# bupt-ai-cz/HIAST

Measured on AMD Instinct MI355X. Metric: self-training images/sec (fwd+bwd+pseudo-label) at 1024x512, higher is better.
Workload: dtype fp16

## Files before the change

hiast_amd/csrc/igemm.hip:

```cpp
#include "igemm_kernel.h"

namespace hiast {

template <int PL>
__device__ __forceinline__ size_t ig_wp_elem(int n, int t, int k, int taps, int KO)
{
    const size_t row = ((size_t)n * taps + t) * PL * KO;
    return PL == 2 ? row + (size_t)(k >> 5) * 64 + (k & 31) : row + k;
}

template <int PL, bool F16 = false>
__global__ __launch_bounds__(256) void pack_conv_weight_kernel(const float* __restrict__ w,
                                                               unsigned short* __restrict__ wp,
                                                               unsigned short* __restrict__ wpt, int N, int K, int taps,
                                                               int mode)
{
    const long long idx = (long long)blockIdx.x * 256 + threadIdx.x;
    if (idx >= (long long)N * taps * K) return;
    const int k = (int)(idx % K);
    const int t = (int)((idx / K) % taps);
    const int n = (int)(idx / ((long long)K * taps));
    const float v = w[((size_t)n * K + k) * taps + t];
    unsigned short h, l = 0;
    if (F16) h = H16<true>::enc(v);
    else ig_split(v, h, l);
    if (mode != 1) {
        unsigned short* d = wp + ig_wp_elem<PL>(n, t, k, taps, K);
        d[0] = h;
        if (PL == 2) d[32] = l;
    }
    if (mode != 0) {
        unsigned short* d = (mode == 1 ? wp : wpt) + ig_wp_elem<PL>(k, taps - 1 - t, n, taps, N);
        d[0] = h;
        if (PL == 2) d[32] = l;
    }
}

constexpr int PK_PITCH = 72;

template <int PL, bool F16 = false>
__device__ __forceinline__ void pack_tile(const float* __restrict__ w, unsigned short* __restrict__ wp,
                                          unsigned short* __restrict__ wpt, int N, int K, int taps, int mode, int n0,
                                          int k0, unsigned short* lds)
{
    constexpr int TN = PL == 1 ? 32 : 16;
    unsigned short* hi = lds;
    unsigned short* lo = lds + (PL == 2 ? TN * taps * PK_PITCH : 0);
    unsigned short* fwd = (mode == 1) ? nullptr : wp;
    unsigned short* adj = (mode == 0) ? nullptr : (mode == 1 ? wp : wpt);
    const int run = 64 * taps;
    for (int nh = 0; nh < 64; nh += TN) {
        if (nh) __syncthreads();
        for (int e = threadIdx.x; e < TN * run; e += 256) {
            const int n = e / run, r = e - n * run;
            const int k = r / taps, t = r - k * taps;
            const float v = w[((size_t)(n0 + nh + n) * K + k0) * taps + r];
            unsigned short h, l = 0;
            if (F16) h = H16<true>::enc(v);
            else ig_split(v, h, l);
            hi[(n * taps + t) * PK_PITCH + k] = h;
            if (PL == 2) lo[(n * taps + t) * PK_PITCH + k] = l;
        }
        __syncthreads();
        if (fwd) {
            for (int e = threadIdx.x; e < TN * taps * 8; e += 256) {
                const int c = e & 7, nt = e >> 3;
                const int n = nt / taps, t = nt - n * taps;
                const uint4 vh = *reinterpret_cast<const uint4*>(&hi[nt * PK_PITCH + c * 8]);
                unsigned short* d = fwd + ig_wp_elem<PL>(n0 + nh + n, t, k0 + c * 8, taps, K);
                *reinterpret_cast<uint4*>(d) = vh;
                if (PL == 2) *reinterpret_cast<uint4*>(d + 32) = *reinterpret_cast<const uint4*>(&lo[nt * PK_PITCH + c * 8]);
            }
        }
        if (adj) {
            for (int e = threadIdx.x; e < 64 * taps * (TN / 8); e += 256) {
                const int c = e % (TN / 8), kt = e / (TN / 8);
                const int k = kt / taps, t = kt - k * taps;
                unsigned short vh[8], vl[8];
#pragma unroll
                for (int j = 0; j < 8; ++j) {
                    vh[j] = hi[((c * 8 + j) * taps + t) * PK_PITCH + k];
                    if (PL == 2) vl[j] = lo[((c * 8 + j) * taps + t) * PK_PITCH + k];
                }
                unsigned short* d = adj + ig_wp_elem<PL>(k0 + k, taps - 1 - t, n0 + nh + c * 8, taps, N);
                *reinterpret_cast<uint4*>(d) = make_uint4(vh[0] | (unsigned)vh[1] << 16, vh[2] | (unsigned)vh[3] << 16,
                                                          vh[4] | (unsigned)vh[5] << 16, vh[6] | (unsigned)vh[7] << 16);
                if (PL == 2)
                    *reinterpret_cast<uint4*>(d + 32) = make_uint4(vl[0] | (unsigned)vl[1] << 16, vl[2] | (unsigned)vl[3] << 16,
                                                                   vl[4] | (unsigned)vl[5] << 16, vl[6] | (unsigned)vl[7] << 16);
            }
        }
    }
}

template <int PL, bool F16 = false>
__global__ __launch_bounds__(256) void pack_conv_weight_tiled_kernel(const float* __restrict__ w,
                                                                     unsigned short* __restrict__ wp,
                                                                     unsigned short* __restrict__ wpt, int N, int K,
                                                                     int taps, int mode)
{
    extern __shared__ __attribute__((aligned(16))) unsigned short lds[];
    const int kt = K / 64;
    pack_tile<PL, F16>(w, wp, wpt, N, K, taps, mode, (int)(blockIdx.x / kt) * 64, (int)(blockIdx.x % kt) * 64, lds);
}

__global__ __launch_bounds__(256) void pack_conv_weight_multi_kernel(const hiast_pack_rec* __restrict__ table,
                                                                     const int32_t* __restrict__ chunk_tensor,
                                                                     const int64_t* __restrict__ chunk_start)
{
    extern __shared__ __attribute__((aligned(16))) unsigned short lds[];
    const hiast_pack_rec r = table[chunk_tensor[blockIdx.x]];
    const int kt = r.K / 64;
    const int tile = (int)chunk_start[blockIdx.x];
    const int n0 = (tile / kt) * 64, k0 = (tile % kt) * 64;
    if (r.planes == HIAST_FMT_SPLIT_BF16)
        pack_tile<2>(r.w, (unsigned short*)r.wp, (unsigned short*)r.wpt, r.N, r.K, r.taps, r.mode, n0, k0, lds);
    else if (r.planes == HIAST_FMT_FP16)
        pack_tile<1, true>(r.w, (unsigned short*)r.wp, (unsigned short*)r.wpt, r.N, r.K, r.taps, r.mode, n0, k0, lds);
    else
        pack_tile<1>(r.w, (unsigned short*)r.wp, (unsigned short*)r.wpt, r.N, r.K, r.taps, r.mode, n0, k0, lds);
}

__global__ __launch_bounds__(256) void to_planes_kernel(const float* __restrict__ x, unsigned short* __restrict__ p,
                                                        long long M, int C)
{
    const long long total8 = M * C / 8;
    for (long long i = (long long)blockIdx.x * 256 + threadIdx.x; i < total8; i += (long long)gridDim.x * 256) {
        const long long m = (i * 8) / C;
        const int c = (int)((i * 8) - m * C);
        const float4 a = reinterpret_cast<const float4*>(x)[2 * i], b = reinterpret_cast<const float4*>(x)[2 * i + 1];
        const float v[8] = {a.x, a.y, a.z, a.w, b.x, b.y, b.z, b.w};
        unsigned ph[4], pl_[4];
#pragma unroll
        for (int q = 0; q < 4; ++q) {
            unsigned short h0, l0, h1, l1;
            ig_split(v[2 * q], h0, l0);
            ig_split(v[2 * q + 1], h1, l1);
            ph[q] = (unsigned)h0 | ((unsigned)h1 << 16);
            pl_[q] = (unsigned)l0 | ((unsigned)l1 << 16);
        }
        unsigned short* dst = p + ig_elem<2>((size_t)m, c, C);
        *reinterpret_cast<uint4*>(dst) = make_uint4(ph[0], ph[1], ph[2], ph[3]);
        *reinterpret_cast<uint4*>(dst + 32) = make_uint4(pl_[0], pl_[1], pl_[2], pl_[3]);
    }
}

__global__ __launch_bounds__(256) void from_planes_kernel(const unsigned short* __restrict__ p, float* __restrict__ x,
                                                          long long M, int C)
{
    const long long total8 = M * C / 8;
    for (long long i = (long long)blockIdx.x * 256 + threadIdx.x; i < total8; i += (long long)gridDim.x * 256) {
        const long long m = (i * 8) / C;
        const int c = (int)((i * 8) - m * C);
        const unsigned short* src = p + ig_elem<2>((size_t)m, c, C);
        const uint4 h = *reinterpret_cast<const uint4*>(src), l = *reinterpret_cast<const uint4*>(src + 32);
        const unsigned wh[4] = {h.x, h.y, h.z, h.w}, wl[4] = {l.x, l.y, l.z, l.w};
        float v[8];
#pragma unroll
        for (int q = 0; q < 4; ++q) {
            v[2 * q] = __uint_as_float(wh[q] << 16) + __uint_as_float(wl[q] << 16);
            v[2 * q + 1] = __uint_as_float(wh[q] & 0xFFFF0000u) + __uint_as_float(wl[q] & 0xFFFF0000u);
        }
        reinterpret_cast<float4*>(x)[2 * i] = make_float4(v[0], v[1], v[2], v[3]);
        reinterpret_cast<float4*>(x)[2 * i + 1] = make_float4(v[4], v[5], v[6], v[7]);
    }
}

}

const IgEnv& hiast_ig_env()
{
    static const IgEnv env = [] {
        IgEnv e;
        const char* v = getenv("HIAST_IGEMM_HALF");
        e.half = v ? (atoi(v) != 0) : -1;
        v = getenv("HIAST_IGEMM_BN");
        const int bn = v ? atoi(v) : 0;
        e.bn = (bn == 64 || bn == 128 || bn == 256) ? bn : 0;
        e.ragged_off = getenv("HIAST_IGEMM_RAGGED") != nullptr;
        v = getenv("HIAST_IGEMM_COSCHED");
        e.cosched0 = v && atoi(v) != 0;
        return e;
    }();
    return env;
}
static thread_local int ig_cosched_tls = -1, ig_half_tls = -1;
int hiast_ig_cosched_tls_get() { return ig_cosched_tls; }
int hiast_ig_half_tls_get() { return ig_half_tls; }
extern "C" int hiast_igemm_set_half(int v)
{
    const int prev = ig_half_tls;
    ig_half_tls = v < 0 ? -1 : (v != 0);
    return prev;
}
extern "C" int hiast_igemm_set_cosched(int on)
{
    const int prev = ig_cosched_tls;
    ig_cosched_tls = on < 0 ? -1 : (on != 0);
    return prev;
}

int hiast_xconv_ok(int64_t M, int K, int N, int planes, int taps, int out_f32, int has_bn, int has_res, int relu,
                   int has_gate, int gate_mask, int has_stats);
int hiast_xconv_stats_rows(int64_t M, int N);
int hiast_xconv_launch(const void* x, const void* wp, const float* gamma, const float* beta, const float* mean,
                       const float* var, float eps, const void* res, int relu, void* y, int64_t M, int K, int N,
                       float* stats, const void* res_gate, int f16, hipStream_t st);
int hiast_xconv2_ok(int64_t M, int K, int N, int planes, int taps, int out_f32, int has_bn, int has_res, int relu,
                    int has_gate, int has_stats);
int hiast_xconv2_launch(const void* x, const void* wp, const float* gamma, const float* beta, const float* mean,
                        const float* var, float eps, const void* res, int relu, void* y, int64_t M, int N, hipStream_t st);
int hiast_igemm_launch_f16(const void* x, const void* wp, const float* gamma, const float* beta, const float* mean,
                           const float* var, float eps, const void* res, int relu, void* y, int64_t M, int K, int N, int taps,
                           hiast::IGeo geo, float* stats, const void* res_gate, int gate_mask, hipStream_t st, int stats_mode,
                           int out_f32, int stats_rows);

static int igemm_launch_mode(const void* x, const void* wp, const float* gamma, const float* beta, const float* mean,
                             const float* var, float eps, const void* res, int relu, void* y, int64_t M, int K, int N,
                             int taps, int H, int W, int stride, int dil, int fmt, int out_f32, hipStream_t st,
                             float* stats, const void* res_gate, int gate_mask, int stats_mode, int stats_rows)
{
    if (!hiast_fmt_ok(fmt)) return HIAST_E_RANGE;
    const int planes = hiast_fmt_planes(fmt), f16 = fmt == HIAST_FMT_FP16;
    if (stats_mode == 2) {
        if (!stats || !res || !mean || !var || planes != 1 || out_f32 || relu || res_gate || N % 8) return HIAST_E_RANGE;
    } else {
        if (stats && (planes != 1 || out_f32 || res || relu)) return HIAST_E_RANGE;
        if ((stats || res_gate) && mean) return HIAST_E_RANGE;
    }
    if (res_gate && (planes != 1 || !res || relu || out_f32 || (!gate_mask && (((uintptr_t)res_gate) & 15)))) return HIAST_E_RANGE;
    if (!x || !wp || !y || (mean && !var)) return HIAST_E_ARG;
    if (M <= 0 || K <= 0 || N <= 0) return HIAST_E_ARG;
    if ((planes != 1 && planes != 2) || (taps != 1 && taps != 9)) return HIAST_E_RANGE;
    if ((K * planes) % 64 != 0 || N % 64 != 0 || M > (1ll << 31) - 512) return HIAST_E_RANGE;
    if (out_f32 && res) return HIAST_E_RANGE;
    if ((((uintptr_t)x) | ((uintptr_t)wp) | ((uintptr_t)y) | ((uintptr_t)res)) & 15) return HIAST_E_RANGE;
    hiast::IGeo geo = {0, 0, 0, 0, 1, 1};
    size_t in_pix = (size_t)M;
    if (taps != 1 && stride == -2) {
        if (H <= 0 || W <= 0 || dil != 1 || planes != 1 || out_f32) return HIAST_E_ARG;
        const int Hs = (H - 1) / 2 + 1, Ws = (W - 1) / 2 + 1;
        if (M % ((int64_t)H * W) != 0) return HIAST_E_ARG;
        geo = {Hs, Ws, H, W, -2, 1};
        in_pix = (size_t)(M / ((int64_t)H * W)) * Hs * Ws;
    } else if (taps != 1) {
        if (H <= 0 || W <= 0 || stride <= 0 || dil <= 0) return HIAST_E_ARG;
        const int Ho = (H - 1) / stride + 1, Wo = (W - 1) / stride + 1;
        if (M % ((int64_t)Ho * Wo) != 0) return HIAST_E_ARG;
        geo = {H, W, Ho, Wo, stride, dil};
        in_pix = (size_t)(M / ((int64_t)Ho * Wo)) * H * W;
    }
    if (in_pix * planes * K * 2 >= (1ull << 31) || (size_t)N * taps * planes * K * 2 >= (1ull << 31)) return HIAST_E_RANGE;
    if (stats_mode != 2 &&
        hiast_xconv_ok(M, K, N, planes, taps, out_f32, mean != nullptr, res != nullptr, relu, res_gate != nullptr, gate_mask,
                       stats != nullptr)) {
        if (stats && stats_rows != hiast_xconv_stats_rows(M, N)) return HIAST_E_ARG;
        return hiast_xconv_launch(x, wp, gamma, beta, mean, var, eps, res, relu, y, M, K, N, stats, res_gate, f16, st);
    }
    if (stats_mode == 0 && !f16 &&
        hiast_xconv2_ok(M, K, N, planes, taps, out_f32, mean != nullptr, res != nullptr, relu, res_gate != nullptr, stats != nullptr))
        return hiast_xconv2_launch(x, wp, gamma, beta, mean, var, eps, res, relu, y, M, N, st);
    if (f16)
        return hiast_igemm_launch_f16(x, wp, gamma, beta, mean, var, eps, res, relu, y, M, K, N, taps, geo, stats, res_gate,
                                      gate_mask, st, stats_mode, out_f32, stats_rows);
    if (planes == 2) {
        if (out_f32) return launch_igemm_t<2, true>(x, wp, gamma, beta, mean, var, eps, res, relu, y, M, K, N, taps, geo, stats, res_gate, gate_mask, st, stats_mode, stats_rows);
        return launch_igemm_t<2, false>(x, wp, gamma, beta, mean, var, eps, res, relu, y, M, K, N, taps, geo, stats, res_gate, gate_mask, st, stats_mode, stats_rows);
    }
    if (out_f32) return launch_igemm_t<1, true>(x, wp, gamma, beta, mean, var, eps, res, relu, y, M, K, N, taps, geo, stats, res_gate, gate_mask, st, stats_mode, stats_rows);
    return launch_igemm_t<1, false>(x, wp, gamma, beta, mean, var, eps, res, relu, y, M, K, N, taps, geo, stats, res_gate, gate_mask, st, stats_mode, stats_rows);
}

int hiast_igemm_launch(const void* x, const void* wp, const float* gamma, const float* beta, const float* mean,
                       const float* var, float eps, const void* res, int relu, void* y, int64_t M, int K, int N,
                       int taps, int H, int W, int stride, int dil, int fmt, int out_f32, hipStream_t st,
                       float* stats, const void* res_gate, int gate_mask, int stats_rows)
{
    return igemm_launch_mode(x, wp, gamma, beta, mean, var, eps, res, relu, y, M, K, N, taps, H, W, stride, dil, fmt,
                             out_f32, st, stats, res_gate, gate_mask, stats ? 1 : 0, stats_rows);
}

extern "C" int hiast_igemm_dgrad_bn_stats(const void* dy, const void* wpt, void* da, int B, int H, int W, int Cin, int Cout,
                                          int taps, int dil, const void* bn_x, const float* gamma, const float* beta,
                                          const float* save_mean, const float* save_invstd, float* partial, int partial_rows,
                                          int fmt, hiast_stream_t stream)
{
    if (fmt != HIAST_FMT_BF16 && fmt != HIAST_FMT_FP16) return HIAST_E_RANGE;
    if (B <= 0 || H <= 0 || W <= 0) return HIAST_E_ARG;
    if (!bn_x || !save_mean || !save_invstd || !partial) return HIAST_E_ARG;
    if ((((uintptr_t)save_mean) | ((uintptr_t)save_invstd) | ((uintptr_t)gamma) | ((uintptr_t)beta)) & 15) return HIAST_E_RANGE;
    return igemm_launch_mode(dy, wpt, gamma, beta, save_mean, save_invstd, 0.0f, bn_x, 0, da, (int64_t)B * H * W, Cin, Cout,
                             taps, H, W, 1, dil, fmt, 0, (hipStream_t)stream, partial, nullptr, 0, 2, partial_rows);
}

extern "C" int hiast_igemm_dgrad_s2(const void* dy, const void* wpt, void* dx, int B, int H, int W, int Cin, int Cout, int fmt,
                                    hiast_stream_t stream)
{
    if (fmt != HIAST_FMT_BF16 && fmt != HIAST_FMT_FP16) return HIAST_E_RANGE;
    if (B <= 0 || H <= 0 || W <= 0) return HIAST_E_ARG;
    return igemm_launch_mode(dy, wpt, nullptr, nullptr, nullptr, nullptr, 0.0f, nullptr, 0, dx, (int64_t)B * H * W, Cout, Cin, 9,
                             H, W, -2, 1, fmt, 0, (hipStream_t)stream, nullptr, nullptr, 0, 0, 0);
}

extern "C" int hiast_igemm_dgrad_bn_stats_rows(int64_t M, int Cin, int Cout, int taps)
{
    if (M <= 0) return 0;
    const int bm = ig_block_rows(M, Cin, Cout, taps, 0);
    return (int)((M + bm - 1) / bm);
}

extern "C" int hiast_igemm_bn_act(const void* x, const void* wp, const float* gamma, const float* beta,
                                  const float* mean, const float* var, float eps, const void* res, int relu, void* y,
                                  int B, int H, int W, int Cin, int Cout, int taps, int stride, int dil, int fmt,
                                  int out_f32, float* stats, int stats_rows, const void* res_gate, int gate_mask,
                                  hiast_stream_t stream)
{
    if (B <= 0 || H <= 0 || W <= 0) return HIAST_E_ARG;
    if (taps == 1 && stride != 1) return HIAST_E_RANGE;
    const int Ho = taps == 1 ? H : (H - 1) / stride + 1, Wo = taps == 1 ? W : (W - 1) / stride + 1;
    return hiast_igemm_launch(x, wp, gamma, beta, mean, var, eps, res, relu, y, (int64_t)B * Ho * Wo, Cin, Cout, taps, H,
                              W, stride, dil, fmt, out_f32, (hipStream_t)stream, stats, res_gate, gate_mask, stats_rows);
}

#ifdef IG_STAMP
namespace hiast {
__global__ void ig_stamp_copy_kernel(unsigned* dst)
{
    for (int i = blockIdx.x * blockDim.x + threadIdx.x; i < 1024 * 8 * 8 + 32 * 64; i += gridDim.x * blockDim.x) dst[i] = ig_stamp_buf[i];
}
}
extern "C" int hiast_igemm_debug_stamps(unsigned* dst_device)
{
    hipLaunchKernelGGL(hiast::ig_stamp_copy_kernel, dim3(64), dim3(256), 0, 0, dst_device);
    return (int)hipDeviceSynchronize();
}
#endif

extern "C" int hiast_igemm_stats_rows(int64_t M, int Cin, int Cout, int taps, int fmt)
{
    const int planes = hiast_fmt_planes(fmt);
    if (M <= 0 || Cin <= 0 || Cout <= 0) return 0;
    if (hiast_xconv_ok(M, Cin, Cout, planes, taps, 0, 0, 0, 0, 0, 0, 1)) return hiast_xconv_stats_rows(M, Cout);
    const int bm = ig_block_rows(M, Cin, Cout, taps, 0);
    return (int)((M + bm - 1) / bm);
}

extern "C" int hiast_pack_conv_weight(const float* w, int N, int K, int taps, int fmt, int transpose, void* wp,
                                      void* wpt, hiast_stream_t stream)
{
    if (!w || !wp) return HIAST_E_ARG;
    if (N <= 0 || K <= 0 || taps <= 0) return HIAST_E_ARG;
    const int planes = fmt;
    if (!hiast_fmt_ok(fmt) || transpose < 0 || transpose > 2) return HIAST_E_RANGE;
    if (transpose == 2 && !wpt) return HIAST_E_ARG;
    const long long total = (long long)N * K * taps;
    if (N % 64 == 0 && K % 64 == 0 && taps <= 9 && !((((uintptr_t)wp) | ((uintptr_t)wpt)) & 15)) {
        const dim3 tg((unsigned)((N / 64) * (K / 64)));
        const size_t lds_bytes = (size_t)32 * taps * hiast::PK_PITCH * sizeof(unsigned short);
        if (planes == HIAST_FMT_SPLIT_BF16)
            hipLaunchKernelGGL(hiast::pack_conv_weight_tiled_kernel<2>, tg, dim3(256), lds_bytes, (hipStream_t)stream, w,
                               (unsigned short*)wp, (unsigned short*)wpt, N, K, taps, transpose);
        else if (planes == HIAST_FMT_FP16)
            hipLaunchKernelGGL((hiast::pack_conv_weight_tiled_kernel<1, true>), tg, dim3(256), lds_bytes, (hipStream_t)stream, w,
                               (unsigned short*)wp, (unsigned short*)wpt, N, K, taps, transpose);
        else
            hipLaunchKernelGGL(hiast::pack_conv_weight_tiled_kernel<1>, tg, dim3(256), lds_bytes, (hipStream_t)stream, w,
                               (unsigned short*)wp, (unsigned short*)wpt, N, K, taps, transpose);
        HIAST_CHECK_LAUNCH();
        return 0;
    }
    const dim3 grid((unsigned)((total + 255) / 256));
    if (planes == HIAST_FMT_SPLIT_BF16)
        hipLaunchKernelGGL(hiast::pack_conv_weight_kernel<2>, grid, dim3(256), 0, (hipStream_t)stream, w,
                           (unsigned short*)wp, (unsigned short*)wpt, N, K, taps, transpose);
    else if (planes == HIAST_FMT_FP16)
        hipLaunchKernelGGL((hiast::pack_conv_weight_kernel<1, true>), grid, dim3(256), 0, (hipStream_t)stream, w,
                           (unsigned short*)wp, (unsigned short*)wpt, N, K, taps, transpose);
    else
        hipLaunchKernelGGL(hiast::pack_conv_weight_kernel<1>, grid, dim3(256), 0, (hipStream_t)stream, w,
                           (unsigned short*)wp, (unsigned short*)wpt, N, K, taps, transpose);
    HIAST_CHECK_LAUNCH();
    return 0;
}

namespace hiast {

template <int INK, int PL, bool F16 = false>
__global__ __launch_bounds__(256) void stem_tail_kernel(const void* __restrict__ xv, const float* __restrict__ gamma,
                                                        const float* __restrict__ beta, const float* __restrict__ mean,
                                                        const float* __restrict__ var, float eps,
                                                        unsigned short* __restrict__ out, int B, int H, int W, int C, int Ho,
                                                        int Wo)
{
    const int G = C >> 3;
    const long long total = (long long)B * Ho * Wo * G;
    const long long stride = (long long)gridDim.x * 256;
    long long i = (long long)blockIdx.x * 256 + threadIdx.x;
    if (i >= total) return;
    const int cg = (int)(i % G);
    float sc[8], sh[8];
#pragma unroll
    for (int k = 0; k < 8; ++k) {
        const int c = cg * 8 + k;
        const float invstd = 1.0f / sqrtf(var[c] + eps);
        sc[k] = (gamma ? gamma[c] : 1.0f) * invstd;
        sh[k] = fmaf(-mean[c], sc[k], beta ? beta[c] : 0.0f);
    }
    for (; i < total; i += stride) {
        const long long pix = i / G;
        const int xo = (int)(pix % Wo);
        const int yo = (int)((pix / Wo) % Ho);
        const int b = (int)(pix / ((long long)Wo * Ho));
        float m[8];
#pragma unroll
        for (int k = 0; k < 8; ++k) m[k] = -INFINITY;
#pragma unroll
        for (int dy = 0; dy < 3; ++dy) {
            const int yy = 2 * yo - 1 + dy;
            if (yy < 0 || yy >= H) continue;
#pragma unroll
            for (int dx = 0; dx < 3; ++dx) {
                const int xx = 2 * xo - 1 + dx;
                if (xx < 0 || xx >= W) continue;
                const size_t off = (((size_t)b * H + yy) * W + xx) * C + cg * 8;
                float v[8];
                if (INK != 0) {
                    const uint4 r = *reinterpret_cast<const uint4*>(reinterpret_cast<const unsigned short*>(xv) + off);
                    const unsigned w4[4] = {r.x, r.y, r.z, r.w};
#pragma unroll
                    for (int q = 0; q < 4; ++q) {
                        v[2 * q] = H16<INK == 2>::lo(w4[q]);
                        v[2 * q + 1] = H16<INK == 2>::hi(w4[q]);
                    }
                } else {
                    const float4 a = *reinterpret_cast<const float4*>(reinterpret_cast<const float*>(xv) + off);
                    const float4 c4 = *reinterpret_cast<const float4*>(reinterpret_cast<const float*>(xv) + off + 4);
                    v[0] = a.x; v[1] = a.y; v[2] = a.z; v[3] = a.w; v[4] = c4.x; v[5] = c4.y; v[6] = c4.z; v[7] = c4.w;
                }
#pragma unroll
                for (int k = 0; k < 8; ++k) {
                    float t = fmaf(v[k], sc[k], sh[k]);
                    t = t > 0.f ? t : 0.f;
                    if (INK != 0) t = H16<INK == 2>::dec(H16<INK == 2>::enc(t));
                    m[k] = t > m[k] ? t : m[k];
                }
            }
        }
        unsigned ph[4], pl_[4];
#pragma unroll
        for (int q = 0; q < 4; ++q) {
            unsigned short h0, l0 = 0, h1, l1 = 0;
            if (PL == 2) {
                ig_split(m[2 * q], h0, l0);
                ig_split(m[2 * q + 1], h1, l1);
            } else {
                h0 = H16<F16>::enc(m[2 * q]);
                h1 = H16<F16>::enc(m[2 * q + 1]);
            }
            ph[q] = (unsigned)h0 | ((unsigned)h1 << 16);
            pl_[q] = (unsigned)l0 | ((unsigned)l1 << 16);
        }
        unsigned short* dst = out + ig_elem<PL>((size_t)pix, cg * 8, C);
        *reinterpret_cast<uint4*>(dst) = make_uint4(ph[0], ph[1], ph[2], ph[3]);
        if (PL == 2) *reinterpret_cast<uint4*>(dst + 32) = make_uint4(pl_[0], pl_[1], pl_[2], pl_[3]);
    }
}

}

extern "C" int hiast_stem_tail(const void* x, int dtype, const float* gamma, const float* beta, const float* mean,
                               const float* var, float eps, void* out, int fmt, int B, int H, int W, int C,
                               hiast_stream_t stream)
{
    if (!hiast_fmt_ok(fmt)) return HIAST_E_RANGE;
    const int planes = hiast_fmt_planes(fmt), f16 = fmt == HIAST_FMT_FP16;
    if (!x || !mean || !var || !out) return HIAST_E_ARG;
    if (B <= 0 || H <= 0 || W <= 0 || C <= 0) return HIAST_E_ARG;
    if (dtype < 0 || dtype > 2 || C % 8 != 0 || (planes == 2 && C % 32 != 0) ||
        ((((uintptr_t)x) | ((uintptr_t)out)) & 15))
        return HIAST_E_RANGE;
    const int Ho = (H - 1) / 2 + 1, Wo = (W - 1) / 2 + 1, G = C / 8;
    const long long total = (long long)B * Ho * Wo * G;
    if ((long long)B * H * W * C >= (1ll << 40)) return HIAST_E_RANGE;
    long long nb = (total + 255) / 256;
    int grid = (int)(nb > 16384 ? 16384 : nb);
    {
        long long a = 256, g = G;
        while (a) { const long long t = g % a; g = a; a = t; }
        const int need = (int)(G / g);
        if (grid >= need) grid -= grid % need;
        else return HIAST_E_RANGE;
    }
    hipStream_t st = (hipStream_t)stream;
#define L(BF, PL)                                                                                                  \
    hipLaunchKernelGGL((hiast::stem_tail_kernel<BF, PL>), dim3(grid), dim3(256), 0, st, x, gamma, beta, mean, var, eps, \
                       (unsigned short*)out, B, H, W, C, Ho, Wo)
#define LF(BF)                                                                                                     \
    hipLaunchKernelGGL((hiast::stem_tail_kernel<BF, 1, true>), dim3(grid), dim3(256), 0, st, x, gamma, beta, mean, var, eps, \
                       (unsigned short*)out, B, H, W, C, Ho, Wo)
    if (f16) { if (dtype == 2) LF(2); else if (dtype == 1) LF(1); else LF(0); }
    else if (dtype == 2) { if (planes == 2) L(2, 2); else L(2, 1); }
    else if (dtype == 1) { if (planes == 2) L(1, 2); else L(1, 1); }
    else { if (planes == 2) L(0, 2); else L(0, 1); }
#undef LF
#undef L
    HIAST_CHECK_LAUNCH();
    return 0;
}

extern "C" int hiast_split_planes(float* x, void* planes, int64_t M, int C, int inverse, hiast_stream_t stream)
{
    if (!x || !planes) return HIAST_E_ARG;
    if (M <= 0 || C <= 0) return HIAST_E_ARG;
    if (C % 32 != 0 || ((((uintptr_t)x) | ((uintptr_t)planes)) & 15)) return HIAST_E_RANGE;
    const long long total8 = (long long)M * C / 8;
    long long nb = (total8 + 255) / 256;
    const int grid = (int)(nb < 1 ? 1 : (nb > 8192 ? 8192 : nb));
    if (inverse)
        hipLaunchKernelGGL(hiast::from_planes_kernel, dim3(grid), dim3(256), 0, (hipStream_t)stream,
                           (const unsigned short*)planes, x, (long long)M, C);
    else
        hipLaunchKernelGGL(hiast::to_planes_kernel, dim3(grid), dim3(256), 0, (hipStream_t)stream, (const float*)x,
                           (unsigned short*)planes, (long long)M, C);
    HIAST_CHECK_LAUNCH();
    return 0;
}

extern "C" int hiast_pack_conv_weight_multi(const hiast_pack_rec* table, const int32_t* chunk_tensor,
                                            const int64_t* chunk_start, int n_chunks, int max_taps, hiast_stream_t stream)
{
    if (!table || !chunk_tensor || !chunk_start) return HIAST_E_ARG;
    if (n_chunks <= 0 || max_taps <= 0) return HIAST_E_ARG;
    if (max_taps > 9) return HIAST_E_RANGE;
    const size_t lds_bytes = (size_t)32 * max_taps * hiast::PK_PITCH * sizeof(unsigned short);
    hipLaunchKernelGGL(hiast::pack_conv_weight_multi_kernel, dim3(n_chunks), dim3(256), lds_bytes, (hipStream_t)stream, table,
                       chunk_tensor, chunk_start);
    HIAST_CHECK_LAUNCH();
    return 0;
}
```

hiast_amd/csrc/xconv.hip:

```cpp
#include <hip/hip_bf16.h>
#include <stdlib.h>

#include "common.h"

namespace hiast {

typedef __attribute__((ext_vector_type(8))) __bf16 xc_bf16x8;
typedef __attribute__((ext_vector_type(4))) float xc_f32x4;
typedef __attribute__((address_space(3))) void* xc_lds_ptr;

constexpr int XC_PANEL = 64;
constexpr int XC_STAGES = 3;
constexpr int XC_COLS = 512;

__device__ __forceinline__ void xc_dma16(__amdgpu_buffer_rsrc_t rs, unsigned char* lds, int voff, int soff)
{
    __builtin_amdgcn_raw_ptr_buffer_load_lds(rs, (xc_lds_ptr)lds, 16, voff, soff, 0, 0);
}

__device__ __forceinline__ int xc_lds_off(int row, int chunk) { return row * 128 + ((chunk ^ ((row >> 1) & 7)) << 4); }


__device__ __forceinline__ xc_bf16x8 xc_lds_read(unsigned addr)
{
    xc_bf16x8 v;
    asm volatile("ds_read_b128 %0, %1" : "=v"(v) : "v"(addr));
    return v;
}
__device__ __forceinline__ void xc_lds_wait(xc_bf16x8& a, xc_bf16x8& b)
{
    asm volatile("s_waitcnt lgkmcnt(0)" : "+v"(a), "+v"(b));
}

__device__ __forceinline__ int xc_chan(int g, int b, int r) { return (b >> 1) * 32 + g * 8 + (b & 1) * 4 + r; }

template <int KC, bool BN, bool RES, bool RELU, bool GATE, bool STATS, bool F16 = false>
__global__ __launch_bounds__(512) void xconv_kernel(const unsigned short* __restrict__ X,
                                                    const unsigned short* __restrict__ Wp,
                                                    const float* __restrict__ gamma, const float* __restrict__ beta,
                                                    const float* __restrict__ mean, const float* __restrict__ var,
                                                    float eps, const unsigned short* __restrict__ R,
                                                    const unsigned char* __restrict__ Rg,
                                                    unsigned short* __restrict__ Y, int M, int N,
                                                    float* __restrict__ stats)
{
    constexpr int SL = KC / 64;
    constexpr int KS = KC / 32;
    constexpr int STAGE = XC_PANEL * KC * 2;
    __shared__ __attribute__((aligned(1024))) unsigned char smem[XC_STAGES * STAGE];
    __shared__ float s_sc[XC_COLS], s_sh[XC_COLS];

    const int tid = threadIdx.x, lane = tid & 63;
    const int wave = __builtin_amdgcn_readfirstlane(tid >> 6);
    const int g = lane >> 4, px = lane & 15;
    const int NG = N / XC_COLS;
    const int xcd = blockIdx.x & 7, slot = blockIdx.x >> 3;
    const int cg = slot % NG;
    const int nstream = (int)gridDim.x / NG;
    const int stream = (slot / NG) * 8 + xcd;
    const int n0 = cg * XC_COLS + wave * 64;
    const int npanel = (M + XC_PANEL - 1) / XC_PANEL;

    xc_bf16x8 wr[4][KS];
#pragma unroll
    for (int b = 0; b < 4; ++b) {
        const unsigned short* wrow = Wp + (size_t)(n0 + xc_chan(px >> 2, b, px & 3)) * KC + g * 8;
#pragma unroll
        for (int s = 0; s < KS; ++s) wr[b][s] = *reinterpret_cast<const xc_bf16x8*>(wrow + s * 32);
    }
#pragma unroll
    for (int b = 0; b < 4; ++b)
#pragma unroll
        for (int s = 0; s < KS; ++s) asm volatile("" : "+v"(wr[b][s]));
    if (BN) {
        for (int c = tid; c < XC_COLS; c += 512) {
            const int n = cg * XC_COLS + c;
            const float sc = (gamma ? gamma[n] : 1.0f) * (1.0f / sqrtf(var[n] + eps));
            s_sc[c] = sc;
            s_sh[c] = fmaf(-mean[n], sc, beta ? beta[n] : 0.0f);
        }
        __syncthreads();
    }

    constexpr int OOB = (int)0x80000000;
    const __amdgpu_buffer_rsrc_t xrs = __builtin_amdgcn_make_buffer_rsrc((void*)X, 0, (int)((size_t)M * KC * 2), 0x00020000);
    const int drow = wave * 8 + (lane >> 3);
    const int dchunk = ((lane & 7) ^ ((drow >> 1) & 7)) * 16;
    auto issue = [&](int p, int st) {
        const int m = p * XC_PANEL + drow;
        const int voff = (p < npanel && m < M) ? (int)((size_t)m * KC * 2) + dchunk : OOB;
        unsigned char* base = smem + st * STAGE + wave * 1024;
#pragma unroll
        for (int j = 0; j < SL; ++j) xc_dma16(xrs, base + j * (XC_PANEL * 128), voff, j * 128);
    };

    const unsigned lds_base = (unsigned)(size_t)smem;
    float st1[STATS ? 16 : 1], st2[STATS ? 16 : 1];
#pragma unroll
    for (int q = 0; q < (STATS ? 16 : 1); ++q) { st1[q] = 0.f; st2[q] = 0.f; }

    issue(stream, 0);
    issue(stream + nstream, 1);
    int it = 0;
    for (int p = stream; p < npanel; p += nstream, ++it) {
        const int st = it % XC_STAGES;
        constexpr int NRES = RES ? (GATE ? 8 : 4) : 0;
        if (it == 0) asm volatile("s_waitcnt vmcnt(%0)\n\ts_barrier" ::"n"(SL) : "memory");
        else asm volatile("s_waitcnt vmcnt(%0)\n\ts_barrier" ::"n"(SL + 8 + NRES) : "memory");
        uint4 rres[RES ? 2 : 1][2];
        unsigned rgate[GATE ? 2 : 1][2];
        auto load_res = [&](int half) {
#pragma unroll
            for (int t = 0; t < 2; ++t) {
                const int m = p * XC_PANEL + half * 32 + t * 16 + px;
                const size_t row = (size_t)(m < M ? m : 0) * N + n0 + g * 8;
                rres[t][0] = h_load16_once(R + row);
                rres[t][1] = h_load16_once(R + row + 32);
                if (GATE) {
                    const unsigned char* gp = Rg + (size_t)(m < M ? m : 0) * (N >> 3) + ((n0 + g * 8) >> 3);
                    rgate[t][0] = gp[0];
                    rgate[t][1] = gp[4];
                }
            }
        };
        if (RES) load_res(0);
        issue(p + 2 * nstream, (it + 2) % XC_STAGES);
#pragma unroll
        for (int half = 0; half < 2; ++half) {
            if (RES && half == 1) load_res(1);
            xc_f32x4 acc[2][4];
#pragma unroll
            for (int a = 0; a < 2; ++a)
#pragma unroll
                for (int b = 0; b < 4; ++b) acc[a][b] = (xc_f32x4){0.f, 0.f, 0.f, 0.f};
            auto frag = [&](int s, int a) {
                return xc_lds_read(lds_base + (unsigned)(st * STAGE + (s >> 1) * (XC_PANEL * 128) +
                                                         xc_lds_off(half * 32 + a * 16 + px, (s & 1) * 4 + g)));
            };
            constexpr bool DB = !(STATS || (BN && RES));
            xc_bf16x8 xa[DB ? 2 : 1][2];
            xa[0][0] = frag(0, 0);
            xa[0][1] = frag(0, 1);
            xc_lds_wait(xa[0][0], xa[0][1]);
#pragma unroll
            for (int s = 0; s < KS; ++s) {
                constexpr int one = DB ? 1 : 0;
                if (DB && s + 1 < KS) {
                    xa[(s + 1) & one][0] = frag(s + 1, 0);
                    xa[(s + 1) & one][1] = frag(s + 1, 1);
                }
#pragma unroll
                for (int a = 0; a < 2; ++a)
#pragma unroll
                    for (int b = 0; b < 4; ++b)
                        acc[a][b] = H16<F16>::mfma16(wr[b][s], xa[s & one][a], acc[a][b]);
                if (s + 1 < KS) {
                    if (!DB) {
                        xa[0][0] = frag(s + 1, 0);
                        xa[0][1] = frag(s + 1, 1);
                    }
                    xc_lds_wait(xa[(s + 1) & one][0], xa[(s + 1) & one][1]);
                }
            }
#pragma unroll
            for (int a = 0; a < 2; ++a) {
                const int m = p * XC_PANEL + half * 32 + a * 16 + px;
                const bool ok = m < M;
                const size_t row = (size_t)(ok ? m : 0) * N + n0 + g * 8;
                const uint4 r0 = rres[RES ? a : 0][0], r1 = rres[RES ? a : 0][1];
                const unsigned gate0 = GATE ? rgate[GATE ? a : 0][0] : 0xFFu;
                const unsigned gate1 = GATE ? rgate[GATE ? a : 0][1] : 0xFFu;
                float o[16];
#pragma unroll
                for (int b = 0; b < 4; ++b)
#pragma unroll
                    for (int r = 0; r < 4; ++r) o[(b >> 1) * 8 + (b & 1) * 4 + r] = acc[a][b][r];
                if (BN) {
#pragma unroll
                    for (int hh = 0; hh < 2; ++hh) {
                        const int c = wave * 64 + hh * 32 + g * 8;
#pragma unroll
                        for (int q = 0; q < 8; q += 4) {
                            const float4 sc = *reinterpret_cast<const float4*>(&s_sc[c + q]);
                            const float4 sh = *reinterpret_cast<const float4*>(&s_sh[c + q]);
                            o[hh * 8 + q] = fmaf(o[hh * 8 + q], sc.x, sh.x);
                            o[hh * 8 + q + 1] = fmaf(o[hh * 8 + q + 1], sc.y, sh.y);
                            o[hh * 8 + q + 2] = fmaf(o[hh * 8 + q + 2], sc.z, sh.z);
                            o[hh * 8 + q + 3] = fmaf(o[hh * 8 + q + 3], sc.w, sh.w);
                        }
                    }
                }
                if (RES) {
                    const unsigned w0[4] = {r0.x, r0.y, r0.z, r0.w}, w1[4] = {r1.x, r1.y, r1.z, r1.w};
#pragma unroll
                    for (int q = 0; q < 4; ++q) {
                        float a0 = H16<F16>::lo(w0[q]), a1 = H16<F16>::hi(w0[q]);
                        float b0 = H16<F16>::lo(w1[q]), b1 = H16<F16>::hi(w1[q]);
                        if (GATE) {
                            a0 = ((gate0 >> (2 * q)) & 1u) ? a0 : 0.f;
                            a1 = ((gate0 >> (2 * q + 1)) & 1u) ? a1 : 0.f;
                            b0 = ((gate1 >> (2 * q)) & 1u) ? b0 : 0.f;
                            b1 = ((gate1 >> (2 * q + 1)) & 1u) ? b1 : 0.f;
                        }
                        o[2 * q] += a0;
                        o[2 * q + 1] += a1;
                        o[8 + 2 * q] += b0;
                        o[8 + 2 * q + 1] += b1;
                    }
                }
                if (RELU) {
#pragma unroll
                    for (int q = 0; q < 16; ++q) o[q] = o[q] > 0.f ? o[q] : 0.f;
                }
                unsigned pk[8];
                if (STATS && F16) {
#pragma unroll
                    for (int q = 0; q < 8; ++q) {
                        pk[q] = H16<F16>::pack(o[2 * q], o[2 * q + 1]);
                        if (ok) {
                            const float v0 = H16<F16>::lo(pk[q]), v1 = H16<F16>::hi(pk[q]);
                            st1[2 * q] += v0; st2[2 * q] = fmaf(v0, v0, st2[2 * q]);
                            st1[2 * q + 1] += v1; st2[2 * q + 1] = fmaf(v1, v1, st2[2 * q + 1]);
                        }
                        __builtin_amdgcn_sched_barrier(0);
                    }
                } else {
#pragma unroll
                    for (int q = 0; q < 8; ++q) pk[q] = H16<F16>::pack(o[2 * q], o[2 * q + 1]);
                    if (STATS && ok) {
#pragma unroll
                        for (int q = 0; q < 8; ++q) {
                            const float v0 = H16<F16>::lo(pk[q]), v1 = H16<F16>::hi(pk[q]);
                            st1[2 * q] += v0; st2[2 * q] = fmaf(v0, v0, st2[2 * q]);
                            st1[2 * q + 1] += v1; st2[2 * q + 1] = fmaf(v1, v1, st2[2 * q + 1]);
                        }
                    }
                }
                if (ok) {
                    h_store16_out(Y + row, pk[0], pk[1], pk[2], pk[3]);
                    h_store16_out(Y + row + 32, pk[4], pk[5], pk[6], pk[7]);
                }
            }
        }
    }
    if (STATS) {
#pragma unroll
        for (int q = 0; q < 16; ++q) {
#pragma unroll
            for (int o = 1; o < 16; o <<= 1) {
                st1[q] += __shfl_xor(st1[q], o, 64);
                st2[q] += __shfl_xor(st2[q], o, 64);
            }
        }
        if (px == 0) {
            float* d = stats + ((size_t)stream * N + n0 + g * 8) * 2;
#pragma unroll
            for (int q = 0; q < 8; ++q) {
                d[2 * q] = st1[q];
                d[2 * q + 1] = st2[q];
                d[64 + 2 * q] = st1[8 + q];
                d[64 + 2 * q + 1] = st2[8 + q];
            }
        }
    }
}

static int xc_blocks(int64_t M, int N)
{
    const int NG = N / XC_COLS;
    const long long npanel = (M + XC_PANEL - 1) / XC_PANEL;
    static const int env_cus = [] { const char* e = getenv("HIAST_XCONV_CUS"); const int v = e ? atoi(e) : 0; return v >= 8 && v <= 256 ? v : 0; }();
    const int cus = env_cus ? env_cus : hiast_grid_cus();
    long long streams = cus / NG / 8 * 8;
    if (streams < 8) streams = 8;
    if (streams > npanel) streams = (npanel + 7) / 8 * 8;
    return (int)(streams * NG);
}

}

int hiast_xconv_ok(int64_t M, int K, int N, int planes, int taps, int out_f32, int has_bn, int has_res, int relu,
                   int has_gate, int gate_mask, int has_stats)
{
    const char* env = getenv("HIAST_XCONV");
    if ((env && atoi(env) == 0) || planes != 1 || taps != 1 || out_f32) return 0;
    if (K != 256 || N % hiast::XC_COLS != 0 || N > 2048) return 0;
    if (has_gate && (!gate_mask || !has_res || relu)) return 0;
    if (has_bn && has_res && !relu) return 0;
    if (has_stats && (has_res || relu || has_bn)) return 0;
    if (M < 4096) return 0;
    return 1;
}

int hiast_xconv_stats_rows(int64_t M, int N)
{
    return hiast::xc_blocks(M, N) / (N / hiast::XC_COLS);
}

int hiast_xconv_launch(const void* x, const void* wp, const float* gamma, const float* beta, const float* mean,
                       const float* var, float eps, const void* res, int relu, void* y, int64_t M, int K, int N,
                       float* stats, const void* res_gate, int f16, hipStream_t st)
{
    using namespace hiast;
    const dim3 grid((unsigned)xc_blocks(M, N));
#define XL(BNF, RESF, RELUF, GATEF, STATSF)                                                                          \
    do {                                                                                                             \
        if (f16)                                                                                                     \
            hipLaunchKernelGGL((xconv_kernel<256, BNF, RESF, RELUF, GATEF, STATSF, true>), grid, dim3(512), 0, st,    \
                               (const unsigned short*)x, (const unsigned short*)wp, gamma, beta, mean, var, eps,      \
                               (const unsigned short*)res, (const unsigned char*)res_gate, (unsigned short*)y, (int)M, N, \
                               stats);                                                                               \
        else                                                                                                         \
            hipLaunchKernelGGL((xconv_kernel<256, BNF, RESF, RELUF, GATEF, STATSF>), grid, dim3(512), 0, st,          \
                               (const unsigned short*)x, (const unsigned short*)wp, gamma, beta, mean, var, eps,      \
                               (const unsigned short*)res, (const unsigned char*)res_gate, (unsigned short*)y, (int)M, N, \
                               stats);                                                                               \
    } while (0)
    const bool bn = mean != nullptr;
    if (stats) { XL(false, false, false, false, true); }
    else if (res_gate) { XL(false, true, false, true, false); }
    else if (res) {
        if (bn) { if (relu) XL(true, true, true, false, false); else return HIAST_E_RANGE; }
        else { if (relu) XL(false, true, true, false, false); else XL(false, true, false, false, false); }
    } else {
        if (bn) { if (relu) XL(true, false, true, false, false); else XL(true, false, false, false, false); }
        else { if (relu) XL(false, false, true, false, false); else XL(false, false, false, false, false); }
    }
#undef XL
    HIAST_CHECK_LAUNCH();
    return 0;
}
```

Baseline: 144.4.

## Extend register-resident-weight xconv kernel to K=512 one-by-one convolutions

Generalizes the xconv 1x1-conv kernel over K through a geometry template. For K=512 it uses 32-column waves with 32-row panels, a reworked DMA slab mapping, stage counts sized to LDS, and a deeper LDS fragment prefetch with counted waits. This moves K=512 1x1 convs, such as ResNet bottleneck layers with enough output channels, off the generic implicit-GEMM path onto the streaming kernel. The cost is more template instantiations and higher register pressure from holding the weights in registers.

```diff
diff --git a/hiast_amd/csrc/igemm.hip b/hiast_amd/csrc/igemm.hip
--- a/hiast_amd/csrc/igemm.hip
+++ b/hiast_amd/csrc/igemm.hip
@@ -202,7 +202,7 @@
 
 int hiast_xconv_ok(int64_t M, int K, int N, int planes, int taps, int out_f32, int has_bn, int has_res, int relu,
                    int has_gate, int gate_mask, int has_stats);
-int hiast_xconv_stats_rows(int64_t M, int N);
+int hiast_xconv_stats_rows(int64_t M, int K, int N);
 int hiast_xconv_launch(const void* x, const void* wp, const float* gamma, const float* beta, const float* mean,
                        const float* var, float eps, const void* res, int relu, void* y, int64_t M, int K, int N,
                        float* stats, const void* res_gate, int f16, hipStream_t st);
@@ -254,7 +254,7 @@
     if (stats_mode != 2 &&
         hiast_xconv_ok(M, K, N, planes, taps, out_f32, mean != nullptr, res != nullptr, relu, res_gate != nullptr, gate_mask,
                        stats != nullptr)) {
-        if (stats && stats_rows != hiast_xconv_stats_rows(M, N)) return HIAST_E_ARG;
+        if (stats && stats_rows != hiast_xconv_stats_rows(M, K, N)) return HIAST_E_ARG;
         return hiast_xconv_launch(x, wp, gamma, beta, mean, var, eps, res, relu, y, M, K, N, stats, res_gate, f16, st);
     }
     if (stats_mode == 0 && !f16 &&
@@ -340,7 +340,7 @@
 {
     const int planes = hiast_fmt_planes(fmt);
     if (M <= 0 || Cin <= 0 || Cout <= 0) return 0;
-    if (hiast_xconv_ok(M, Cin, Cout, planes, taps, 0, 0, 0, 0, 0, 0, 1)) return hiast_xconv_stats_rows(M, Cout);
+    if (hiast_xconv_ok(M, Cin, Cout, planes, taps, 0, 0, 0, 0, 0, 0, 1)) return hiast_xconv_stats_rows(M, Cin, Cout);
     const int bm = ig_block_rows(M, Cin, Cout, taps, 0);
     return (int)((M + bm - 1) / bm);
 }
diff --git a/hiast_amd/csrc/xconv.hip b/hiast_amd/csrc/xconv.hip
--- a/hiast_amd/csrc/xconv.hip
+++ b/hiast_amd/csrc/xconv.hip
@@ -9,9 +9,26 @@
 typedef __attribute__((ext_vector_type(4))) float xc_f32x4;
 typedef __attribute__((address_space(3))) void* xc_lds_ptr;
 
-constexpr int XC_PANEL = 64;
-constexpr int XC_STAGES = 3;
-constexpr int XC_COLS = 512;
+#ifndef XC_K512_PANEL
+#define XC_K512_PANEL 32
+#endif
+
+template <int KC>
+struct XcGeo {
+    static constexpr int WC = 64 * 256 / KC;
+    static constexpr int NB = WC / 16;
+    static constexpr int HH = NB / 2;
+    static constexpr int COLS = 8 * WC;
+    static constexpr int PANEL = KC == 256 ? 64 : XC_K512_PANEL;
+    static constexpr int STAGE = PANEL * KC * 2;
+    static constexpr int STAGES = 3 * STAGE <= 96 * 1024 ? 3 : 2;
+    static constexpr int AHEAD = STAGES - 1;
+    static constexpr int HALVES = PANEL / 32;
+    static constexpr int DMAS = STAGE / 1024 / 8;
+    static_assert(NB == 2 || NB == 4, "xconv: K is 256 or 512");
+    static_assert(PANEL == 32 || PANEL == 64, "xconv: panels of 32 or 64 rows");
+    static_assert(STAGES * STAGE <= 128 * 1024, "xconv: LDS");
+};
 
 __device__ __forceinline__ void xc_dma16(__amdgpu_buffer_rsrc_t rs, unsigned char* lds, int voff, int soff)
 {
@@ -30,6 +47,11 @@
 __device__ __forceinline__ void xc_lds_wait(xc_bf16x8& a, xc_bf16x8& b)
 {
     asm volatile("s_waitcnt lgkmcnt(0)" : "+v"(a), "+v"(b));
+}
+template <int N>
+__device__ __forceinline__ void xc_lds_wait_n(xc_bf16x8& a, xc_bf16x8& b)
+{
+    asm volatile("s_waitcnt lgkmcnt(%2)" : "+v"(a), "+v"(b) : "n"(N));
 }
 
 __device__ __forceinline__ int xc_chan(int g, int b, int r) { return (b >> 1) * 32 + g * 8 + (b & 1) * 4 + r; }
@@ -44,9 +66,10 @@
                                                     unsigned short* __restrict__ Y, int M, int N,
                                                     float* __restrict__ stats)
 {
-    constexpr int SL = KC / 64;
+    using G = XcGeo<KC>;
     constexpr int KS = KC / 32;
-    constexpr int STAGE = XC_PANEL * KC * 2;
+    constexpr int NB = G::NB, HH = G::HH, WC = G::WC;
+    constexpr int XC_PANEL = G::PANEL, XC_STAGES = G::STAGES, XC_COLS = G::COLS, STAGE = G::STAGE;
     __shared__ __attribute__((aligned(1024))) unsigned char smem[XC_STAGES * STAGE];
     __shared__ float s_sc[XC_COLS], s_sh[XC_COLS];
 
@@ -58,18 +81,18 @@
     const int cg = slot % NG;
     const int nstream = (int)gridDim.x / NG;
     const int stream = (slot / NG) * 8 + xcd;
-    const int n0 = cg * XC_COLS + wave * 64;
+    const int n0 = cg * XC_COLS + wave * WC;
     const int npanel = (M + XC_PANEL - 1) / XC_PANEL;
 
-    xc_bf16x8 wr[4][KS];
-#pragma unroll
-    for (int b = 0; b < 4; ++b) {
+    xc_bf16x8 wr[NB][KS];
+#pragma unroll
+    for (int b = 0; b < NB; ++b) {
         const unsigned short* wrow = Wp + (size_t)(n0 + xc_chan(px >> 2, b, px & 3)) * KC + g * 8;
 #pragma unroll
         for (int s = 0; s < KS; ++s) wr[b][s] = *reinterpret_cast<const xc_bf16x8*>(wrow + s * 32);
     }
 #pragma unroll
-    for (int b = 0; b < 4; ++b)
+    for (int b = 0; b < NB; ++b)
 #pragma unroll
         for (int s = 0; s < KS; ++s) asm volatile("" : "+v"(wr[b][s]));
     if (BN) {
@@ -83,60 +106,90 @@
     }
 
     constexpr int OOB = (int)0x80000000;
+    constexpr int RG = XC_PANEL / 8, SLW = G::DMAS;
     const __amdgpu_buffer_rsrc_t xrs = __builtin_amdgcn_make_buffer_rsrc((void*)X, 0, (int)((size_t)M * KC * 2), 0x00020000);
-    const int drow = wave * 8 + (lane >> 3);
+    const int drow = (wave % RG) * 8 + (lane >> 3);
+    const int dslab = wave / RG;
     const int dchunk = ((lane & 7) ^ ((drow >> 1) & 7)) * 16;
     auto issue = [&](int p, int st) {
         const int m = p * XC_PANEL + drow;
-        const int voff = (p < npanel && m < M) ? (int)((size_t)m * KC * 2) + dchunk : OOB;
-        unsigned char* base = smem + st * STAGE + wave * 1024;
-#pragma unroll
-        for (int j = 0; j < SL; ++j) xc_dma16(xrs, base + j * (XC_PANEL * 128), voff, j * 128);
+        const int voff = (p < npanel && m < M) ? (int)((size_t)m * KC * 2) + dslab * 128 + dchunk : OOB;
+        unsigned char* base = smem + st * STAGE + dslab * (XC_PANEL * 128) + (wave % RG) * 1024;
+#pragma unroll
+        for (int j = 0; j < SLW; ++j) xc_dma16(xrs, base + j * (8 / RG) * (XC_PANEL * 128), voff, j * (8 / RG) * 128);
     };
 
     const unsigned lds_base = (unsigned)(size_t)smem;
-    float st1[STATS ? 16 : 1], st2[STATS ? 16 : 1];
-#pragma unroll
-    for (int q = 0; q < (STATS ? 16 : 1); ++q) { st1[q] = 0.f; st2[q] = 0.f; }
-
-    issue(stream, 0);
-    issue(stream + nstream, 1);
+    float st1[STATS ? 4 * NB : 1], st2[STATS ? 4 * NB : 1];
+#pragma unroll
+    for (int q = 0; q < (STATS ? 4 * NB : 1); ++q) { st1[q] = 0.f; st2[q] = 0.f; }
+
+#pragma unroll
+    for (int a = 0; a < G::AHEAD; ++a) issue(stream + a * nstream, a);
     int it = 0;
     for (int p = stream; p < npanel; p += nstream, ++it) {
         const int st = it % XC_STAGES;
-        constexpr int NRES = RES ? (GATE ? 8 : 4) : 0;
-        if (it == 0) asm volatile("s_waitcnt vmcnt(%0)\n\ts_barrier" ::"n"(SL) : "memory");
-        else asm volatile("s_waitcnt vmcnt(%0)\n\ts_barrier" ::"n"(SL + 8 + NRES) : "memory");
-        uint4 rres[RES ? 2 : 1][2];
-        unsigned rgate[GATE ? 2 : 1][2];
+        constexpr int NRES = RES ? (GATE ? 2 * NB : NB) : 0;
+        constexpr int TAIL = G::HALVES * NB + (G::HALVES - 1) * NRES;
+        static_assert(SLW + TAIL < 64, "xconv: vmcnt is a 6-bit counter");
+        if (it == 0) asm volatile("s_waitcnt vmcnt(%0)\n\ts_barrier" ::"n"(G::AHEAD == 2 ? SLW : 0) : "memory");
+        else asm volatile("s_waitcnt vmcnt(%0)\n\ts_barrier" ::"n"(G::AHEAD == 2 ? SLW + TAIL : TAIL) : "memory");
+        uint4 rres[RES ? 2 : 1][HH];
+        unsigned rgate[GATE ? 2 : 1][HH];
         auto load_res = [&](int half) {
 #pragma unroll
             for (int t = 0; t < 2; ++t) {
                 const int m = p * XC_PANEL + half * 32 + t * 16 + px;
                 const size_t row = (size_t)(m < M ? m : 0) * N + n0 + g * 8;
-                rres[t][0] = h_load16_once(R + row);
-                rres[t][1] = h_load16_once(R + row + 32);
+#pragma unroll
+                for (int hh = 0; hh < HH; ++hh) rres[t][hh] = h_load16_once(R + row + hh * 32);
                 if (GATE) {
                     const unsigned char* gp = Rg + (size_t)(m < M ? m : 0) * (N >> 3) + ((n0 + g * 8) >> 3);
-                    rgate[t][0] = gp[0];
-                    rgate[t][1] = gp[4];
+#pragma unroll
+                    for (int hh = 0; hh < HH; ++hh) rgate[t][hh] = gp[hh * 4];
                 }
             }
         };
         if (RES) load_res(0);
-        issue(p + 2 * nstream, (it + 2) % XC_STAGES);
-#pragma unroll
-        for (int half = 0; half < 2; ++half) {
+        issue(p + G::AHEAD * nstream, (it + G::AHEAD) % XC_STAGES);
+#pragma unroll
+        for (int half = 0; half < G::HALVES; ++half) {
             if (RES && half == 1) load_res(1);
-            xc_f32x4 acc[2][4];
+            xc_f32x4 acc[2][NB];
 #pragma unroll
             for (int a = 0; a < 2; ++a)
 #pragma unroll
-                for (int b = 0; b < 4; ++b) acc[a][b] = (xc_f32x4){0.f, 0.f, 0.f, 0.f};
+                for (int b = 0; b < NB; ++b) acc[a][b] = (xc_f32x4){0.f, 0.f, 0.f, 0.f};
             auto frag = [&](int s, int a) {
                 return xc_lds_read(lds_base + (unsigned)(st * STAGE + (s >> 1) * (XC_PANEL * 128) +
                                                          xc_lds_off(half * 32 + a * 16 + px, (s & 1) * 4 + g)));
             };
+            if constexpr (NB == 2) {
+                constexpr int PF = 3;
+                xc_bf16x8 xr[PF + 1][2];
+#pragma unroll
+                for (int q = 0; q < PF; ++q) {
+                    xr[q][0] = frag(q, 0);
+                    xr[q][1] = frag(q, 1);
+                }
+#pragma unroll
+                for (int s = 0; s < KS; ++s) {
+                    if (s + PF < KS) {
+                        xr[(s + PF) % (PF + 1)][0] = frag(s + PF, 0);
+                        xr[(s + PF) % (PF + 1)][1] = frag(s + PF, 1);
+                    }
+                    const int younger = KS - 1 - s < PF ? KS - 1 - s : PF;
+                    if (younger == 3) xc_lds_wait_n<6>(xr[s % (PF + 1)][0], xr[s % (PF + 1)][1]);
+                    else if (younger == 2) xc_lds_wait_n<4>(xr[s % (PF + 1)][0], xr[s % (PF + 1)][1]);
+                    else if (younger == 1) xc_lds_wait_n<2>(xr[s % (PF + 1)][0], xr[s % (PF + 1)][1]);
+                    else xc_lds_wait_n<0>(xr[s % (PF + 1)][0], xr[s % (PF + 1)][1]);
+#pragma unroll
+                    for (int a = 0; a < 2; ++a)
+#pragma unroll
+                        for (int b = 0; b < NB; ++b)
+                            acc[a][b] = H16<F16>::mfma16(wr[b][s], xr[s % (PF + 1)][a], acc[a][b]);
+                }
+            } else {
             constexpr bool DB = !(STATS || (BN && RES));
             xc_bf16x8 xa[DB ? 2 : 1][2];
             xa[0][0] = frag(0, 0);
@@ -152,7 +205,7 @@
 #pragma unroll
                 for (int a = 0; a < 2; ++a)
 #pragma unroll
-                    for (int b = 0; b < 4; ++b)
+                    for (int b = 0; b < NB; ++b)
                         acc[a][b] = H16<F16>::mfma16(wr[b][s], xa[s & one][a], acc[a][b]);
                 if (s + 1 < KS) {
                     if (!DB) {
@@ -162,23 +215,21 @@
                     xc_lds_wait(xa[(s + 1) & one][0], xa[(s + 1) & one][1]);
                 }
             }
+            }
 #pragma unroll
             for (int a = 0; a < 2; ++a) {
                 const int m = p * XC_PANEL + half * 32 + a * 16 + px;
                 const bool ok = m < M;
                 const size_t row = (size_t)(ok ? m : 0) * N + n0 + g * 8;
-                const uint4 r0 = rres[RES ? a : 0][0], r1 = rres[RES ? a : 0][1];
-                const unsigned gate0 = GATE ? rgate[GATE ? a : 0][0] : 0xFFu;
-                const unsigned gate1 = GATE ? rgate[GATE ? a : 0][1] : 0xFFu;
-                float o[16];
-#pragma unroll
-                for (int b = 0; b < 4; ++b)
+                float o[4 * NB];
+#pragma unroll
+                for (int b = 0; b < NB; ++b)
 #pragma unroll
                     for (int r = 0; r < 4; ++r) o[(b >> 1) * 8 + (b & 1) * 4 + r] = acc[a][b][r];
                 if (BN) {
 #pragma unroll
-                    for (int hh = 0; hh < 2; ++hh) {
-                        const int c = wave * 64 + hh * 32 + g * 8;
+                    for (int hh = 0; hh < HH; ++hh) {
+                        const int c = wave * WC + hh * 32 + g * 8;
 #pragma unroll
                         for (int q = 0; q < 8; q += 4) {
                             const float4 sc = *reinterpret_cast<const float4*>(&s_sc[c + q]);
@@ -191,31 +242,31 @@
                     }
                 }
                 if (RES) {
-                    const unsigned w0[4] = {r0.x, r0.y, r0.z, r0.w}, w1[4] = {r1.x, r1.y, r1.z, r1.w};
-#pragma unroll
-                    for (int q = 0; q < 4; ++q) {
-                        float a0 = H16<F16>::lo(w0[q]), a1 = H16<F16>::hi(w0[q]);
-                        float b0 = H16<F16>::lo(w1[q]), b1 = H16<F16>::hi(w1[q]);
-                        if (GATE) {
-                            a0 = ((gate0 >> (2 * q)) & 1u) ? a0 : 0.f;
-                            a1 = ((gate0 >> (2 * q + 1)) & 1u) ? a1 : 0.f;
-                            b0 = ((gate1 >> (2 * q)) & 1u) ? b0 : 0.f;
-                            b1 = ((gate1 >> (2 * q + 1)) & 1u) ? b1 : 0.f;
+#pragma unroll
+                    for (int hh = 0; hh < HH; ++hh) {
+                        const uint4 r = rres[RES ? a : 0][hh];
+                        const unsigned gate = GATE ? rgate[GATE ? a : 0][hh] : 0xFFu;
+                        const unsigned w[4] = {r.x, r.y, r.z, r.w};
+#pragma unroll
+                        for (int q = 0; q < 4; ++q) {
+                            float a0 = H16<F16>::lo(w[q]), a1 = H16<F16>::hi(w[q]);
+                            if (GATE) {
+                                a0 = ((gate >> (2 * q)) & 1u) ? a0 : 0.f;
+                                a1 = ((gate >> (2 * q + 1)) & 1u) ? a1 : 0.f;
+                            }
+                            o[hh * 8 + 2 * q] += a0;
+                            o[hh * 8 + 2 * q + 1] += a1;
                         }
-                        o[2 * q] += a0;
-                        o[2 * q + 1] += a1;
-                        o[8 + 2 * q] += b0;
-                        o[8 + 2 * q + 1] += b1;
                     }
                 }
                 if (RELU) {
 #pragma unroll
-                    for (int q = 0; q < 16; ++q) o[q] = o[q] > 0.f ? o[q] : 0.f;
-                }
-                unsigned pk[8];
+                    for (int q = 0; q < 4 * NB; ++q) o[q] = o[q] > 0.f ? o[q] : 0.f;
+                }
+                unsigned pk[2 * NB];
                 if (STATS && F16) {
 #pragma unroll
-                    for (int q = 0; q < 8; ++q) {
+                    for (int q = 0; q < 2 * NB; ++q) {
                         pk[q] = H16<F16>::pack(o[2 * q], o[2 * q + 1]);
                         if (ok) {
                             const float v0 = H16<F16>::lo(pk[q]), v1 = H16<F16>::hi(pk[q]);
@@ -226,10 +277,10 @@
                     }
                 } else {
 #pragma unroll
-                    for (int q = 0; q < 8; ++q) pk[q] = H16<F16>::pack(o[2 * q], o[2 * q + 1]);
+                    for (int q = 0; q < 2 * NB; ++q) pk[q] = H16<F16>::pack(o[2 * q], o[2 * q + 1]);
                     if (STATS && ok) {
 #pragma unroll
-                        for (int q = 0; q < 8; ++q) {
+                        for (int q = 0; q < 2 * NB; ++q) {
                             const float v0 = H16<F16>::lo(pk[q]), v1 = H16<F16>::hi(pk[q]);
                             st1[2 * q] += v0; st2[2 * q] = fmaf(v0, v0, st2[2 * q]);
                             st1[2 * q + 1] += v1; st2[2 * q + 1] = fmaf(v1, v1, st2[2 * q + 1]);
@@ -237,15 +288,16 @@
                     }
                 }
                 if (ok) {
-                    h_store16_out(Y + row, pk[0], pk[1], pk[2], pk[3]);
-                    h_store16_out(Y + row + 32, pk[4], pk[5], pk[6], pk[7]);
+#pragma unroll
+                    for (int hh = 0; hh < HH; ++hh)
+                        h_store16_out(Y + row + hh * 32, pk[4 * hh], pk[4 * hh + 1], pk[4 * hh + 2], pk[4 * hh + 3]);
                 }
             }
         }
     }
     if (STATS) {
 #pragma unroll
-        for (int q = 0; q < 16; ++q) {
+        for (int q = 0; q < 4 * NB; ++q) {
 #pragma unroll
             for (int o = 1; o < 16; o <<= 1) {
                 st1[q] += __shfl_xor(st1[q], o, 64);
@@ -255,20 +307,23 @@
         if (px == 0) {
             float* d = stats + ((size_t)stream * N + n0 + g * 8) * 2;
 #pragma unroll
-            for (int q = 0; q < 8; ++q) {
-                d[2 * q] = st1[q];
-                d[2 * q + 1] = st2[q];
-                d[64 + 2 * q] = st1[8 + q];
-                d[64 + 2 * q + 1] = st2[8 + q];
-            }
+            for (int hh = 0; hh < HH; ++hh)
+#pragma unroll
+                for (int q = 0; q < 8; ++q) {
+                    d[hh * 64 + 2 * q] = st1[hh * 8 + q];
+                    d[hh * 64 + 2 * q + 1] = st2[hh * 8 + q];
+                }
         }
     }
 }
 
-static int xc_blocks(int64_t M, int N)
-{
-    const int NG = N / XC_COLS;
-    const long long npanel = (M + XC_PANEL - 1) / XC_PANEL;
+static int xc_cols(int K) { return K == 512 ? XcGeo<512>::COLS : XcGeo<256>::COLS; }
+
+static int xc_blocks(int64_t M, int N, int K)
+{
+    const int NG = N / xc_cols(K);
+    const int panel = K == 512 ? XcGeo<512>::PANEL : XcGeo<256>::PANEL;
+    const long long npanel = (M + panel - 1) / panel;
     static const int env_cus = [] { const char* e = getenv("HIAST_XCONV_CUS"); const int v = e ? atoi(e) : 0; return v >= 8 && v <= 256 ? v : 0; }();
     const int cus = env_cus ? env_cus : hiast_grid_cus();
     long long streams = cus / NG / 8 * 8;
@@ -284,7 +339,8 @@
 {
     const char* env = getenv("HIAST_XCONV");
     if ((env && atoi(env) == 0) || planes != 1 || taps != 1 || out_f32) return 0;
-    if (K != 256 || N % hiast::XC_COLS != 0 || N > 2048) return 0;
+    if ((K != 256 && K != 512) || N % hiast::xc_cols(K) != 0 || N > 2048) return 0;
+    if (K == 512 && (N < 512 || (has_gate && N < 2048))) return 0;
     if (has_gate && (!gate_mask || !has_res || relu)) return 0;
     if (has_bn && has_res && !relu) return 0;
     if (has_stats && (has_res || relu || has_bn)) return 0;
@@ -292,9 +348,9 @@
     return 1;
 }
 
-int hiast_xconv_stats_rows(int64_t M, int N)
-{
-    return hiast::xc_blocks(M, N) / (N / hiast::XC_COLS);
+int hiast_xconv_stats_rows(int64_t M, int K, int N)
+{
+    return hiast::xc_blocks(M, N, K) / (N / hiast::xc_cols(K));
 }
 
 int hiast_xconv_launch(const void* x, const void* wp, const float* gamma, const float* beta, const float* mean,
@@ -302,19 +358,21 @@
                        float* stats, const void* res_gate, int f16, hipStream_t st)
 {
     using namespace hiast;
-    const dim3 grid((unsigned)xc_blocks(M, N));
+    if (K != 256 && K != 512) return HIAST_E_RANGE;
+    const dim3 grid((unsigned)xc_blocks(M, N, K));
+#define XK(KCF, BNF, RESF, RELUF, GATEF, STATSF, F16F)                                                               \
+    hipLaunchKernelGGL((xconv_kernel<KCF, BNF, RESF, RELUF, GATEF, STATSF, F16F>), grid, dim3(512), 0, st,            \
+                       (const unsigned short*)x, (const unsigned short*)wp, gamma, beta, mean, var, eps,              \
+                       (const unsigned short*)res, (const unsigned char*)res_gate, (unsigned short*)y, (int)M, N, stats)
 #define XL(BNF, RESF, RELUF, GATEF, STATSF)                                                                          \
     do {                                                                                                             \
-        if (f16)                                                                                                     \
-            hipLaunchKernelGGL((xconv_kernel<256, BNF, RESF, RELUF, GATEF, STATSF, true>), grid, dim3(512), 0, st,    \
-                               (const unsigned short*)x, (const unsigned short*)wp, gamma, beta, mean, var, eps,      \
-                               (const unsigned short*)res, (const unsigned char*)res_gate, (unsigned short*)y, (int)M, N, \
-                               stats);                                                                               \
-        else                                                                                                         \
-            hipLaunchKernelGGL((xconv_kernel<256, BNF, RESF, RELUF, GATEF, STATSF>), grid, dim3(512), 0, st,          \
-                               (const unsigned short*)x, (const unsigned short*)wp, gamma, beta, mean, var, eps,      \
-                               (const unsigned short*)res, (const unsigned char*)res_gate, (unsigned short*)y, (int)M, N, \
-                               stats);                                                                               \
+        if (K == 512) {                                                                                              \
+            if (f16) XK(512, BNF, RESF, RELUF, GATEF, STATSF, true);                                                 \
+            else XK(512, BNF, RESF, RELUF, GATEF, STATSF, false);                                                    \
+        } else {                                                                                                     \
+            if (f16) XK(256, BNF, RESF, RELUF, GATEF, STATSF, true);                                                 \
+            else XK(256, BNF, RESF, RELUF, GATEF, STATSF, false);                                                    \
+        }                                                                                                            \
     } while (0)
     const bool bn = mean != nullptr;
     if (stats) { XL(false, false, false, false, true); }
@@ -327,6 +385,7 @@
         else { if (relu) XL(false, false, true, false, false); else XL(false, false, false, false, false); }
     }
 #undef XL
+#undef XK
     HIAST_CHECK_LAUNCH();
     return 0;
 }
```

Result: no change. 143.1 (-0.9%).
